# pyani-plus/pyani-plus

Measured on AMD Instinct MI355X. Metric: pairwise genome comparisons/sec (N x N ANI matrix), higher is better.
Workload: dtype u64

## Files before the change

### include/pyani_hip.h

```cpp
#ifndef PYANI_HIP_H
#define PYANI_HIP_H

#include <stddef.h>
#include <stdint.h>

#ifdef __cplusplus
extern "C" {
#endif

#define PA_ABI_VERSION 5

#define PA_API __attribute__((visibility("default")))

typedef enum pa_status {
  PA_OK = 0,
  PA_E_INVALID = -1,
  PA_E_HIP = -2,
  PA_E_NOMEM = -3,
  PA_E_CAPACITY = -4,
  PA_E_NODEVICE = -5,
  PA_E_IO = -6,
  PA_E_NOCONVERGE = -7
} pa_status;

// ... 31 lines not shown
PA_API int pa_fasta_batch_load(const char *const *paths, uint32_t n, int threads, pa_fasta_batch **out);
PA_API int pa_fasta_batch_info(const pa_fasta_batch *batch, uint32_t i, char md5hex33[33], uint64_t *n_residues,
                        uint64_t *n_records, uint64_t *n_invalid, uint64_t *n_bases, uint64_t *n_text,
                        const char **description, const char **message, int *was_gzip);
PA_API int pa_fasta_batch_records(const pa_fasta_batch *batch, uint32_t i, const uint64_t **rec_start,
                           const uint64_t **rec_len, uint64_t *n_records);
PA_API uint64_t pa_fasta_batch_arena_bases(const pa_fasta_batch *batch);
PA_API int pa_fasta_batch_copy_arena(const pa_fasta_batch *batch, uint32_t *h_packed, uint32_t *h_mask,
                              uint64_t *h_genome_start);
PA_API void pa_fasta_batch_free(pa_fasta_batch *batch);

PA_API uint64_t pa_max_hash(uint64_t scaled);

PA_API int pa_arena_dirty(pa_ctx *ctx, const uint32_t *d_mask, uint64_t arena_bases, uint64_t *d_dirty);

PA_API int pa_sketch(pa_ctx *ctx, const uint32_t *d_packed, const uint32_t *d_mask, const uint64_t *d_dirty,
              uint64_t arena_bases, const uint64_t *h_genome_start, uint32_t n_genomes, uint32_t k, uint64_t max_hash,
              uint64_t *d_hashes, uint64_t cap_hashes, uint64_t *d_off, uint64_t *h_total);

PA_API int64_t pa_mask_runs(const uint32_t *h_mask, uint64_t arena_bases, uint64_t *h_run_start, uint64_t *h_run_len,
                            uint64_t cap);
PA_API int pa_mask_from_runs(pa_ctx *ctx, const uint64_t *h_run_start, const uint64_t *h_run_len, uint32_t n_runs,
                             uint32_t *d_mask, uint64_t arena_bases);
PA_API int pa_sketch_streamed(pa_ctx *ctx, const uint32_t *h_packed, const uint64_t *h_run_start,
                              const uint64_t *h_run_len, uint32_t n_runs, uint64_t arena_bases,
                              const uint64_t *h_genome_start, uint32_t n_genomes, uint32_t k, uint64_t max_hash,
                              uint32_t *d_packed, uint32_t *d_mask, uint64_t *d_dirty, uint64_t *d_hashes,
                              uint64_t cap_hashes, uint64_t *d_off, uint64_t *h_total);

#define PA_PAIRS_AUTO 0
#define PA_PAIRS_BITROW 1
#define PA_PAIRS_MERGE 2
#define PA_PAIRS_BITROW_HASH 3
PA_API int pa_pair_counts(pa_ctx *ctx, const uint64_t *d_hashes, const uint64_t *d_off, uint32_t n,
                   uint32_t q0, uint32_t q1, uint32_t s0, uint32_t s1, uint32_t *d_counts, int algo);
PA_API int pa_pair_counts_ex(pa_ctx *ctx, const uint64_t *d_hashes, const uint64_t *d_off, const uint64_t *h_off,
                      uint32_t n, uint32_t q0, uint32_t q1, uint32_t s0, uint32_t s1, uint32_t *d_counts, int algo);
PA_API int pa_pair_dict_prepare(pa_ctx *ctx, const uint64_t *d_subject_hashes, uint64_t n_postings);

PA_API int pa_ani(pa_ctx *ctx, const uint32_t *d_counts, const uint64_t *d_off, uint32_t q0, uint32_t q1,
           uint32_t s0, uint32_t s1, uint32_t k, double *d_identity, double *d_cov_query);
PA_API int pa_ani_host(const uint32_t *h_counts, const uint64_t *h_q_sizes, const uint64_t *h_s_sizes,
                uint32_t nq, uint32_t ns, uint32_t k, double *h_identity, double *h_cov_query,
                uint8_t *h_is_null, int symmetric, uint32_t n_threads);

PA_API int pa_sketch_bottom(pa_ctx *ctx, const uint32_t *d_packed, const uint32_t *d_mask, const uint64_t *d_dirty, uint64_t arena_bases,
                     const uint64_t *h_genome_start, uint32_t n_genomes, uint32_t k, uint32_t m, uint64_t *d_hashes,
                     uint64_t cap_hashes, uint64_t *d_off, uint64_t *h_total);
PA_API int pa_pair_mash(pa_ctx *ctx, const uint64_t *d_hashes, const uint64_t *d_off, uint32_t n, uint32_t q0, uint32_t q1,
                 uint32_t s0, uint32_t s1, uint32_t m, uint32_t *d_common, uint32_t *d_denom);
PA_API int pa_ani_mash(pa_ctx *ctx, const uint32_t *d_common, const uint32_t *d_denom, uint64_t n_pairs, uint32_t k,
                double *d_ani);

PA_API int pa_fragani(pa_ctx *ctx, const uint32_t *d_packed, const uint32_t *d_mask, uint64_t arena_bases,
               const uint64_t *h_contig_start, const uint32_t *h_contig_len, const uint32_t *h_contig_genome,
               uint32_t n_contigs, uint32_t n_genomes, uint32_t k, uint32_t frag_len, uint32_t ref0, uint32_t ref1,
               uint32_t *h_total_frags, uint32_t *h_matched, double *h_ident_sum);
#define PA_FRAGANI_REUSE_INDEX 1u
#define PA_FRAGANI_COLUMNS_ONLY 2u
PA_API int pa_fragani_ex(pa_ctx *ctx, const uint32_t *d_packed, const uint32_t *d_mask, uint64_t arena_bases,
                  const uint64_t *h_contig_start, const uint32_t *h_contig_len, const uint32_t *h_contig_genome,
                  uint32_t n_contigs, uint32_t n_genomes, uint32_t k, uint32_t frag_len, uint32_t qry0, uint32_t qry1,
                  uint32_t ref0, uint32_t ref1, uint32_t flags, uint32_t *h_total_frags, uint32_t *h_matched,
                  double *h_ident_sum);
PA_API int pa_fragani_workspace(pa_ctx *ctx, uint64_t *held_bytes, uint64_t *peak_bytes, uint64_t *cap_bytes);
PA_API int pa_fragani_set_workspace_cap(pa_ctx *ctx, uint64_t cap_bytes);
// ... 231 lines not shown
```

### pyani_plus_amd/_capi.py

```python

from __future__ import annotations

import ctypes as C
import os
import subprocess
from pathlib import Path

_PKG = Path(__file__).resolve().parent
LIB_PATH = _PKG / "_lib" / "libpyani_hip.so"
TOOLS_LIB_PATH = _PKG / "_lib" / "libpyani_hip_tools.so"

ABI_VERSION = 5
PA_OK = 0
PA_E_INVALID = -1
PA_E_NOMEM = -3
PA_E_CAPACITY = -4
PA_E_IO = -6
PA_E_NOCONVERGE = -7
PA_MUL_TALL_MAX_P = 32
PA_EIGS_MAX_K = 24
PA_MANTEL_MAX_N = 16384
PA_MANTEL_LANES = 64
PA_MANTEL_BATCH = 256
PA_MSA_BOOT_BATCH = 32
PA_DEREP_GREEDY, PA_DEREP_COVER = 0, 1
PA_DEREP_MODE = {"greedy": PA_DEREP_GREEDY, "cover": PA_DEREP_COVER}
PA_DEREP_BATCH = 64
PA_DEREP_NONE = 0xFFFFFFFF
PA_SIG_UNHANDLED = 1
PA_FRAGANI_REUSE_INDEX = 1
PA_FRAGANI_COLUMNS_ONLY = 2
PA_PAIRS_AUTO, PA_PAIRS_BITROW, PA_PAIRS_MERGE, PA_PAIRS_BITROW_HASH = 0, 1, 2, 3
PA_ALIGN_BASES = 64
PA_SELECT_MAX_RANKS = 8
PA_KDE_CHAIN = 2048
PA_HIST_WIDE_LDS_BINS = 8192
PA_BIN2D_MAX_BINS = 1024
PA_BIN2D_LDS_CELLS = 4096
PA_BIN2D_SLOTS = 2048
PA_BIN2D_NONE = 0xFFFFFFFFFFFFFFFF
PA_TETRA_BINS = 336
PA_TETRA_WORDS = 256
PROF_PHASES = {"kmer_hash": 0, "sketch_sort": 1, "pair_dict": 2, "pair_count": 3, "ani": 4, "frag_index": 5, "frag_seed": 6, "frag_map": 7,
               "msa_pack": 8, "msa_pairs": 9, "cls_edges": 10, "cls_sort": 11, "rowdist": 12, "nj_scan": 13, "nj_join": 14, "nj_update": 15,
               "msa_boot": 16, "msa_boot_dist": 17}
PA_AGG = {"min": 0, "max": 1, "mean": 2}

_u8p = C.POINTER(C.c_uint8)
_u32p = C.POINTER(C.c_uint32)
_u64p = C.POINTER(C.c_uint64)
_f64p = C.POINTER(C.c_double)
_vp = C.c_void_p

SIGNATURES: dict[str, tuple] = {
    "pa_abi_version": (C.c_int, []),
    "pa_last_error": (C.c_char_p, []),
    "pa_device_count": (C.c_int, []),
    "pa_ctx_create": (C.c_int, [C.c_int, C.POINTER(_vp)]),
    "pa_ctx_destroy": (None, [_vp]),
    "pa_ctx_set_stream": (C.c_int, [_vp, _vp]),
    "pa_ctx_own_stream": (C.c_int, [_vp]),
    "pa_ctx_sync": (C.c_int, [_vp]),
    "pa_ctx_device_info": (C.c_int, [_vp, C.c_char_p, C.POINTER(C.c_int), _u64p]),
    "pa_dev_alloc": (C.c_int, [_vp, C.c_uint64, C.POINTER(_vp)]),
    "pa_dev_free": (C.c_int, [_vp, _vp]),
# ... 233 lines not shown
```

### pyani_plus_amd/csrc/capi.hip

```cpp
#include <algorithm>
#include <cstdarg>
#include <cstring>

#include "pa_internal.h"

static thread_local char g_err[1024] = "";

void pa_set_error(const char *fmt, ...) {
  va_list ap;
  va_start(ap, fmt);
  vsnprintf(g_err, sizeof(g_err), fmt, ap);
  va_end(ap);
}

static hipEvent_t take_event(pa_ctx *c) {
  if (!c->event_pool.empty()) {
    hipEvent_t e = c->event_pool.back();
    c->event_pool.pop_back();
    return e;
  }
  hipEvent_t e = nullptr;
  if (hipEventCreate(&e) != hipSuccess) return nullptr;
  return e;
}
// ... 232 lines not shown
    uint64_t *keys[2] = {c->cand_keys[0].as<uint64_t>(), c->cand_keys[1].as<uint64_t>()};
    uint32_t *vals[2] = {c->cand_vals[0].as<uint32_t>(), c->cand_vals[1].as<uint32_t>()};
    int which = 0;
    int hash_bits = max_hash ? 64 - __builtin_clzll(max_hash) : 0;
    hash_bits = (hash_bits + 7) & ~7;
    int genome_bits = n_genomes > 1 ? 32 - __builtin_clz(n_genomes - 1) : 0;
    genome_bits = (genome_bits + 7) & ~7;
    PA_TRY(pa_radix_sort_pairs(c, keys, vals, n_cand, 0, hash_bits, false, &which));
    PA_TRY(pa_radix_sort_pairs(c, keys, vals, n_cand, 0, genome_bits, true, &which));
    int st = pa_build_sketch_csr(c, keys[which], vals[which], n_cand, n_genomes, d_hashes, cap_hashes, d_off, h_total);
    if (st != PA_OK) return st;
  }
  return PA_OK;
}

extern "C" {

int pa_sketch(pa_ctx *c, const uint32_t *d_packed, const uint32_t *d_mask, const uint64_t *d_dirty_in, uint64_t arena_bases,
              const uint64_t *h_genome_start, uint32_t n_genomes, uint32_t k, uint64_t max_hash, uint64_t *d_hashes,
              uint64_t cap_hashes, uint64_t *d_off, uint64_t *h_total) {
  PA_REQUIRE(c && d_off && h_total && h_genome_start, "pa_sketch: null argument");
  PA_REQUIRE(arena_bases == 0 || (d_packed && d_mask), "pa_sketch: null arena");
  SketchPlan plan;
  PA_TRY(pa_sketch_plan(h_genome_start, n_genomes, arena_bases, k, max_hash, "pa_sketch", &plan));
  PA_HIP(hipSetDevice(c->device));
  return pa_sketch_resident(c, d_packed, d_mask, d_dirty_in, plan, k, max_hash, d_hashes, cap_hashes, d_off, h_total);
}

int pa_pair_counts_ex(pa_ctx *c, const uint64_t *d_hashes, const uint64_t *d_off, const uint64_t *h_off, uint32_t n,
                      uint32_t q0, uint32_t q1, uint32_t s0, uint32_t s1, uint32_t *d_counts, int algo) {
  PA_REQUIRE(c && d_off, "pa_pair_counts: null argument");
  PA_REQUIRE(q0 <= q1 && q1 <= n && s0 <= s1 && s1 <= n, "pa_pair_counts: ranges [%u,%u) x [%u,%u) outside [0,%u)", q0,
             q1, s0, s1, n);
  PA_REQUIRE(algo == PA_PAIRS_AUTO || algo == PA_PAIRS_BITROW || algo == PA_PAIRS_MERGE || algo == PA_PAIRS_BITROW_HASH,
             "pa_pair_counts: unknown algo %d", algo);
  PA_HIP(hipSetDevice(c->device));
  if (q0 == q1 || s0 == s1) { c->dict_prepared = false; return PA_OK; }
  PA_REQUIRE(d_counts != nullptr, "pa_pair_counts: null counts buffer");
  uint64_t total = 0;
  if (h_off) {
    total = h_off[n];
  } else {
    PA_TRY(pa_read_back(c, d_off + n, &total));
  }
  PA_REQUIRE(total == 0 || d_hashes, "pa_pair_counts: null hashes");
  if (algo != PA_PAIRS_AUTO && algo != PA_PAIRS_BITROW_HASH) c->dict_prepared = false;
  switch (algo) {
    case PA_PAIRS_AUTO:
    case PA_PAIRS_BITROW_HASH:
      return pa_pairs_bitrow_hash(c, d_hashes, d_off, h_off, n, total, q0, q1, s0, s1, d_counts);
    case PA_PAIRS_BITROW:
      return pa_pairs_bitrow(c, d_hashes, d_off, n, total, q0, q1, s0, s1, d_counts);
    case PA_PAIRS_MERGE:
      return pa_pairs_merge(c, d_hashes, d_off, n, q0, q1, s0, s1, d_counts);
    default:
      pa_set_error("pa_pair_counts: unknown algo %d", algo);
      return PA_E_INVALID;
  }
}

int pa_pair_counts(pa_ctx *c, const uint64_t *d_hashes, const uint64_t *d_off, uint32_t n, uint32_t q0, uint32_t q1,
                   uint32_t s0, uint32_t s1, uint32_t *d_counts, int algo) {
  return pa_pair_counts_ex(c, d_hashes, d_off, nullptr, n, q0, q1, s0, s1, d_counts, algo);
}

int pa_pair_dict_prepare(pa_ctx *c, const uint64_t *d_subject_hashes, uint64_t n_postings) {
  PA_REQUIRE(c && (n_postings == 0 || d_subject_hashes), "pa_pair_dict_prepare: null argument");
  PA_HIP(hipSetDevice(c->device));
  return pa_pair_dict_prepare_impl(c, d_subject_hashes, n_postings);
}

int pa_ani(pa_ctx *c, const uint32_t *d_counts, const uint64_t *d_off, uint32_t q0, uint32_t q1, uint32_t s0,
           uint32_t s1, uint32_t k, double *d_identity, double *d_cov_query) {
  PA_REQUIRE(c && d_counts && d_off && d_identity && d_cov_query, "pa_ani: null argument");
  PA_REQUIRE(k >= 1 && q0 <= q1 && s0 <= s1, "pa_ani: bad k or ranges");
  PA_HIP(hipSetDevice(c->device));
  return pa_launch_ani(c, d_counts, d_off, q0, q1, s0, s1, k, d_identity, d_cov_query);
}

int pa_prof_enable(pa_ctx *c, int on) {
  PA_REQUIRE(c != nullptr, "null context");
  c->prof_on = on != 0;
  return PA_OK;
// ... 57 lines not shown
```

### pyani_plus_amd/csrc/pa_internal.h

```cpp
#pragma once

#include <hip/hip_runtime.h>

#include <algorithm>
#include <cstdarg>
#include <cstdint>
#include <cstdio>
#include <cstring>
#include <initializer_list>
#include <string>
#include <type_traits>
#include <vector>

#include "../../include/pyani_hip.h"
#include "pa_launch_geom.h"

void pa_set_error(const char *fmt, ...);

#define PA_HIP(call)                                                                          \
  do {                                                                                        \
    hipError_t _e = (call);                                                                   \
    if (_e != hipSuccess) {                                                                   \
      pa_set_error("%s failed: %s (%s:%d)", #call, hipGetErrorString(_e), __FILE__, __LINE__); \
      return PA_E_HIP;                                                                        \
// ... 78 lines not shown

struct ScalarSlot {
  uint32_t word, words;
  constexpr uint32_t bytes() const { return words * 4u; }
  constexpr bool apart_from(ScalarSlot o) const { return word + words <= o.word || o.word + o.words <= word; }
};
constexpr bool slots_apart(uint32_t region_bytes, std::initializer_list<ScalarSlot> slots) {
  for (const ScalarSlot *a = slots.begin(); a != slots.end(); ++a) {
    if ((a->word + a->words) * 4u > region_bytes || (a->words % 2 == 0 && a->word % 2)) return false;
    for (const ScalarSlot *b = a + 1; b != slots.end(); ++b)
      if (!a->apart_from(*b)) return false;
  }
  return true;
}

constexpr uint32_t kCtxScalarBytes = 128;
constexpr ScalarSlot kCandCount{0, 2};
constexpr ScalarSlot kSketchTotal{2, 2};
constexpr ScalarSlot kDenseIds{4, 4};
constexpr uint32_t kDenseOr = 0, kDenseDistinct = 1;
constexpr ScalarSlot kCompactTotal{8, 2};
constexpr ScalarSlot kRegionOverflow{12, 1};
constexpr ScalarSlot kNjPick{16, 8};
constexpr ScalarSlot kDistBad{24, 8};
constexpr ScalarSlot kDerepProgress{14, 2};
static_assert(slots_apart(kCtxScalarBytes, {kCandCount, kSketchTotal, kDenseIds, kCompactTotal, kRegionOverflow, kNjPick, kDistBad, kDerepProgress}),
              "two slots of pa_ctx::counters overlap or leave the block");

constexpr uint32_t kDictScalarBytes = 64;
constexpr ScalarSlot kDictCounters{0, 2};
constexpr uint32_t kDictIdCounter = 0, kDictSpecialId = 1;
constexpr ScalarSlot kDictPreparedFp{2, 4};
constexpr ScalarSlot kDictTileFp{6, 4};
static_assert(slots_apart(kDictScalarBytes, {kDictCounters, kDictPreparedFp, kDictTileFp}),
              "two slots of pa_ctx::dict_scalars overlap or leave the block");

constexpr uint32_t kPinnedBytes = 64;

#define PA_CTX_BUFFERS(ONE, PAIR)                                                                                   \
  PAIR(cand_keys) PAIR(cand_vals) ONE(genome_blk) ONE(counters) ONE(hist) ONE(flags) ONE(scan_tmp) ONE(region_off) \
  ONE(region_cursor) ONE(dirty) PAIR(dict_keys) PAIR(dict_vals) ONE(ids) ONE(post_genome) ONE(bitrows)             \
  ONE(dict_scalars) ONE(cls_i) ONE(cls_j) ONE(cls_score) ONE(cls_cov) ONE(bin2d) ONE(tetra_tab) ONE(nj_work) ONE(pcoa_work) \
  ONE(mantel_work) ONE(derep_work) ONE(boot_work)

struct pa_ctx {
  int device = 0;
  hipStream_t stream = nullptr;
  bool own_stream = false;
  hipDeviceProp_t prop;
#define PA_ONE(name) DevBuf name;
#define PA_PAIR(name) DevBuf name[2];
  PA_CTX_BUFFERS(PA_ONE, PA_PAIR)
#undef PA_ONE
#undef PA_PAIR
  template <class Fn>
  void each_buffer(Fn &&fn) {
#define PA_ONE(name) fn(name);
#define PA_PAIR(name) fn(name[0]); fn(name[1]);
    PA_CTX_BUFFERS(PA_ONE, PA_PAIR)
#undef PA_ONE
#undef PA_PAIR
  }
  template <typename T = uint32_t>
  T *slot(ScalarSlot s) const { return reinterpret_cast<T *>(counters.as<uint32_t>() + s.word); }
  template <typename T = uint32_t>
  T *dict_slot(ScalarSlot s) const { return reinterpret_cast<T *>(dict_scalars.as<uint32_t>() + s.word); }
  bool dict_prepared = false;
  uint64_t dict_prepared_postings = 0;
  uint32_t dict_prepared_cap = 0;
  hipStream_t copy_stream = nullptr;
  void *frag_work = nullptr;
  uint64_t *h_pinned = nullptr;
  bool prof_on = false;
  ProfPhase prof[PA_PROF_NPHASES];
  std::vector<hipEvent_t> event_pool;
// ... 152 lines not shown
      const uint64_t room = (uint64_t)((double)(h_genome_start[g + 1] - s) * plan->frac * 1.25) + 128;
      plan->longest_region = std::max(plan->longest_region, room);
      plan->region_off[g + 1] = plan->region_off[g] + room;
    }
  }
  PA_REQUIRE(plan->n_blocks < (1ULL << 32), "%s: arena too large", who);
  return PA_OK;
}
int pa_regions_begin(pa_ctx *c, const SketchPlan &plan);
CandSink pa_region_sink(pa_ctx *c, uint32_t n_genomes);
int pa_sketch_resident(pa_ctx *c, const uint32_t *d_packed, const uint32_t *d_mask, const uint64_t *d_dirty_in,
                       const SketchPlan &plan, uint32_t k, uint64_t max_hash, uint64_t *d_hashes, uint64_t cap_hashes,
                       uint64_t *d_off, uint64_t *h_total);

int pa_build_dirty(pa_ctx *c, const uint32_t *d_mask, uint64_t n_blocks64, uint64_t *d_dirty, hipStream_t stream = nullptr);
int pa_dirty_or_build(pa_ctx *c, const uint32_t *d_mask, uint64_t n_blocks64, const uint64_t *d_dirty, const uint64_t **out);

constexpr uint32_t kLdsSortMax = 16384;
int pa_sketch_from_regions(pa_ctx *c, uint64_t *d_regions, const uint64_t *d_region_off, const uint32_t *d_cursor,
                           const uint32_t *d_overflow, uint32_t n_genomes, uint32_t longest_region, uint64_t max_hash,
                           uint64_t *d_hashes, uint64_t cap_hashes, uint64_t *d_off, uint64_t *h_total, bool *h_overflow);

int pa_build_sketch_csr(pa_ctx *c, const uint64_t *d_sorted_hash, const uint32_t *d_sorted_genome,
                        uint64_t n_cand, uint32_t n_genomes, uint64_t *d_hashes, uint64_t cap_hashes,
                        uint64_t *d_off, uint64_t *h_total);

int pa_pairs_bitrow(pa_ctx *c, const uint64_t *d_hashes, const uint64_t *d_off, uint32_t n, uint64_t total,
                    uint32_t q0, uint32_t q1, uint32_t s0, uint32_t s1, uint32_t *d_counts);
int pa_dense_ids_sorted(pa_ctx *c, const uint64_t *d_hashes, const uint64_t *d_off, uint32_t n, uint64_t P,
                        uint64_t *n_distinct);
int pa_pairs_bitrow_hash(pa_ctx *c, const uint64_t *d_hashes, const uint64_t *d_off, const uint64_t *h_off ,
                         uint32_t n, uint64_t total, uint32_t q0, uint32_t q1, uint32_t s0, uint32_t s1,
                         uint32_t *d_counts);
int pa_pair_dict_prepare_impl(pa_ctx *c, const uint64_t *d_subject_hashes, uint64_t n_postings);
int pa_pairs_merge(pa_ctx *c, const uint64_t *d_hashes, const uint64_t *d_off, uint32_t n, uint32_t q0,
                   uint32_t q1, uint32_t s0, uint32_t s1, uint32_t *d_counts);

int pa_launch_ani(pa_ctx *c, const uint32_t *d_counts, const uint64_t *d_off, uint32_t q0, uint32_t q1,
                  uint32_t s0, uint32_t s1, uint32_t k, double *d_identity, double *d_cov_query);
```

### pyani_plus_amd/csrc/pairs_bitrow.hip

```cpp
#include <algorithm>
#include <cstdlib>
#include <vector>

#include "pa_internal.h"

namespace {

constexpr int kThreads = 256;
constexpr int kPlanes = 10;
constexpr uint32_t kMaxTileSubjects = 2048;
constexpr uint32_t kNone = 0xffffffffu;
constexpr uint64_t kEmptyKey = ~0ULL;

__global__ __launch_bounds__(kThreads) void iota_kernel(uint32_t *__restrict__ vals, uint64_t n) {
  const uint64_t i = (uint64_t)blockIdx.x * kThreads + threadIdx.x;
  if (i < n) vals[i] = (uint32_t)i;
}

__global__ __launch_bounds__(kThreads) void last_or_kernel(const uint64_t *__restrict__ hashes,
                                                           const uint64_t *__restrict__ off, uint32_t n,
                                                           unsigned long long *__restrict__ or_out) {
  const uint32_t g = blockIdx.x * kThreads + threadIdx.x;
  uint64_t k = 0;
  if (g < n && off[g + 1] > off[g]) k = hashes[off[g + 1] - 1];
// ... 204 lines not shown

template <bool SET_BITS>
__global__ __launch_bounds__(kThreads) void table_lookup_kernel(
    const uint64_t *__restrict__ hashes, uint64_t p0, uint64_t p1, const DictEntry *__restrict__ table, uint32_t cap,
    const uint32_t *__restrict__ special, uint32_t *__restrict__ ids_csr, const uint64_t *__restrict__ off, uint32_t n,
    uint32_t t0, uint32_t w32, uint32_t *__restrict__ rows) {
  uint64_t p;
  if constexpr (SET_BITS) {
    const uint64_t beg = off[t0 + blockIdx.y];
    p = beg + (uint64_t)blockIdx.x * kThreads + threadIdx.x;
    if (p >= off[t0 + blockIdx.y + 1]) return;
  } else {
    p = p0 + (uint64_t)blockIdx.x * kThreads + threadIdx.x;
    if (p >= p1) return;
  }
  const uint64_t h = hashes[p];
  uint32_t id = kNone;
  if (h == kEmptyKey) {
    id = special[0];
  } else {
    uint32_t slot = slot_of(h, cap);
    for (;;) {
      const uint4 e = *reinterpret_cast<const uint4 *>(&table[slot]);
      const uint64_t k = ((uint64_t)e.y << 32) | e.x;
      if (k == h) { id = e.z; break; }
      if (k == kEmptyKey) break;
      if (++slot == cap) slot = 0;
    }
  }
  ids_csr[p] = id;
  if constexpr (SET_BITS) {
    const uint32_t col = blockIdx.y;
    atomicOr(&rows[(uint64_t)id * w32 + (col >> 5)], 1u << (col & 31u));
  }
}

__global__ __launch_bounds__(kThreads) void postings_fingerprint_kernel(const uint64_t *__restrict__ hashes, uint64_t n,
                                                                        unsigned long long *__restrict__ out) {
  uint64_t a = 0, b = 0;
  for (uint64_t i = (uint64_t)blockIdx.x * kThreads + threadIdx.x; i < n; i += (uint64_t)gridDim.x * kThreads) {
    const uint64_t h = hashes[i];
    a += h;
    b += (h ^ (h >> 29)) * 0x9E3779B97F4A7C15ULL;
  }
#pragma unroll
  for (int o = 32; o > 0; o >>= 1) { a += __shfl_xor(a, o, 64); b += __shfl_xor(b, o, 64); }
  if ((threadIdx.x & 63u) == 0) {
    atomicAdd(&out[0], (unsigned long long)a);
    atomicAdd(&out[1], (unsigned long long)b);
  }
}

__global__ __launch_bounds__(256) void mirror_lower_kernel(uint32_t *__restrict__ counts, uint32_t n, uint32_t tile) {
  __shared__ uint32_t s_t[32][33];
  const uint32_t r0 = blockIdx.y * 32u, c0 = blockIdx.x * 32u;
  if (r0 / tile <= c0 / tile) return;
  const uint32_t tx = threadIdx.x & 31u, ty = threadIdx.x >> 5;
  for (uint32_t y = ty; y < 32u; y += 8u) {
    const uint32_t sr = c0 + y, sc = r0 + tx;
    s_t[y][tx] = (sr < n && sc < n) ? counts[(uint64_t)sr * n + sc] : 0u;
  }
  __syncthreads();
  for (uint32_t y = ty; y < 32u; y += 8u) {
    const uint32_t dr = r0 + y, dc = c0 + tx;
    if (dr < n && dc < n) counts[(uint64_t)dr * n + dc] = s_t[tx][y];
  }
// ... 87 lines not shown


static int dict_insert(pa_ctx *c, const uint64_t *d_postings, uint64_t n_post, uint32_t *cap_out) {
  const uint64_t cap64 = n_post + n_post / 2 + 1024;
  PA_REQUIRE(cap64 < (1ULL << 32), "pair phase: tile with %llu subject postings is too large for the hash dictionary",
             (unsigned long long)n_post);
  PA_TRY(c->dict_scalars.reserve(kDictScalarBytes));
  uint32_t *d_counter = c->dict_slot(kDictCounters) + kDictIdCounter, *d_special = c->dict_slot(kDictCounters) + kDictSpecialId;
  PA_TRY(c->dict_keys[0].reserve(cap64 * sizeof(DictEntry)));
  PA_HIP(hipMemsetAsync(c->dict_keys[0].p, 0xff, cap64 * sizeof(DictEntry), c->stream));
  PA_HIP(hipMemsetAsync(d_counter, 0, 4, c->stream));
  PA_HIP(hipMemsetAsync(d_special, 0xff, 4, c->stream));
  PA_TRY(PA_LAUNCH(c, table_insert_kernel, ceil_div(n_post, kThreads * kInsertPerThread), kThreads, 0, d_postings, (uint64_t)0, n_post,
                   c->dict_keys[0].as<DictEntry>(), (uint32_t)cap64, d_counter, d_special));
  *cap_out = (uint32_t)cap64;
  return PA_OK;
}

int pa_pair_dict_prepare_impl(pa_ctx *c, const uint64_t *d_subject_hashes, uint64_t n_postings) {
  ProfScope prof(c, PA_PROF_PAIR_DICT);
  c->dict_prepared = false;
  uint32_t cap = 0;
  PA_TRY(dict_insert(c, d_subject_hashes, n_postings, &cap));
  unsigned long long *d_fp = c->dict_slot<unsigned long long>(kDictPreparedFp);
  PA_HIP(hipMemsetAsync(d_fp, 0, kDictPreparedFp.bytes(), c->stream));
  PA_TRY(PA_LAUNCH(c, postings_fingerprint_kernel, std::min<uint64_t>(1024u, ceil_div(n_postings, kThreads)), kThreads, 0, d_subject_hashes,
                   n_postings, d_fp));
  c->dict_prepared = true;
  c->dict_prepared_postings = n_postings;
  c->dict_prepared_cap = cap;
  return PA_OK;
}

int pa_pairs_bitrow_hash(pa_ctx *c, const uint64_t *d_hashes, const uint64_t *d_off, const uint64_t *h_off_in,
                         uint32_t n, uint64_t total, uint32_t q0, uint32_t q1, uint32_t s0, uint32_t s1,
                         uint32_t *d_counts) {
  const uint32_t nq = q1 - q0, ns = s1 - s0;
  const bool prepared = c->dict_prepared;
  c->dict_prepared = false;
  if (nq == 0 || ns == 0) return PA_OK;
  if (total == 0) {
    PA_HIP(hipMemsetAsync(d_counts, 0, (uint64_t)nq * ns * sizeof(uint32_t), c->stream));
    return PA_OK;
  }
  PA_REQUIRE(total < (1ULL << 32), "pair phase: %llu postings exceed the 32-bit index space", (unsigned long long)total);
  std::vector<uint64_t> h_off_own;
  const uint64_t *h_off = h_off_in;
  if (!h_off) {
    h_off_own.resize(n + 1);
    PA_TRY(pa_copy_to_host(c, h_off_own.data(), d_off, (uint64_t)(n + 1) * 8));
    h_off = h_off_own.data();
  }
  PA_TRY(c->ids.reserve(total * sizeof(uint32_t)));
  PA_TRY(c->dict_scalars.reserve(kDictScalarBytes));
  uint32_t *d_ids = c->ids.as<uint32_t>();
  uint32_t *d_counter = c->dict_slot(kDictCounters) + kDictIdCounter, *d_special = c->dict_slot(kDictCounters) + kDictSpecialId;
  PA_REQUIRE(!prepared || ns <= kMaxTileSubjects, "pair phase: a prepared dictionary serves one tile of at most %u subjects",
             kMaxTileSubjects);
  static const bool symmetry_off = [] { const char *v = PA_TOOL_ENV("PA_PAIRS_SYMMETRIC"); return v && v[0] == '0'; }();
  const bool symmetric = !symmetry_off && q0 == s0 && q1 == s1 && ns > kMaxTileSubjects;
  for (uint32_t t0 = s0; t0 < s1; t0 += kMaxTileSubjects) {
    const uint32_t t1 = (s1 - t0 > kMaxTileSubjects) ? t0 + kMaxTileSubjects : s1;
    const uint32_t cols = t1 - t0;
    const int tpr = (int)((cols + 127u) / 128u);
    const uint32_t w32 = (uint32_t)tpr * 4u;
    const uint32_t tq1 = symmetric ? t1 : q1;
    const uint64_t pt0 = h_off[t0], pt1 = h_off[t1], pq0 = h_off[q0], pq1 = h_off[tq1];
    uint32_t cap = 0;
    {
      ProfScope prof(c, PA_PROF_PAIR_DICT);
      if (prepared) {
        PA_REQUIRE(c->dict_prepared_postings == pt1 - pt0,
                   "pair phase: the prepared dictionary holds %llu postings, the subject tile has %llu",
                   (unsigned long long)c->dict_prepared_postings, (unsigned long long)(pt1 - pt0));
        unsigned long long *d_tile_fp = c->dict_slot<unsigned long long>(kDictTileFp);
        PA_HIP(hipMemsetAsync(d_tile_fp, 0, kDictTileFp.bytes(), c->stream));
        PA_TRY(PA_LAUNCH(c, postings_fingerprint_kernel, std::min<uint64_t>(1024u, ceil_div(pt1 - pt0, kThreads)), kThreads, 0, d_hashes + pt0,
                         pt1 - pt0, d_tile_fp));
        unsigned long long fp_prepared[2], fp_tile[2];
        ReadBack rb(c);
        PA_TRY(rb.queue(c->dict_slot<unsigned long long>(kDictPreparedFp), fp_prepared, 2));
        PA_TRY(rb.queue(d_tile_fp, fp_tile, 2));
        PA_TRY(rb.wait());
        PA_REQUIRE(fp_prepared[0] == fp_tile[0] && fp_prepared[1] == fp_tile[1],
                   "pair phase: the prepared dictionary was built from other postings than the subject tile's "
                   "(same count, %llu, different content)", (unsigned long long)(pt1 - pt0));
        cap = c->dict_prepared_cap;
      } else {
        PA_TRY(dict_insert(c, d_hashes + pt0, pt1 - pt0, &cap));
      }
      constexpr uint64_t kRowBoundBytes = 4ULL << 30;
      uint64_t row_bound = (pt1 - pt0) ? (pt1 - pt0) : 1;
      if (row_bound * w32 * sizeof(uint32_t) > kRowBoundBytes && row_bound * w32 * sizeof(uint32_t) > c->bitrows.bytes) {
        uint32_t distinct = 0;
        PA_TRY(pa_read_back(c, d_counter, &distinct));
        row_bound = std::max<uint64_t>(1, std::min<uint64_t>(row_bound, distinct));
      }
      PA_TRY(c->bitrows.reserve(row_bound * w32 * sizeof(uint32_t)));
      PA_TRY(PA_LAUNCH(c, zero_rows_kernel, ceil_div(row_bound * w32 / 4u, kThreads), kThreads, 0, c->bitrows.as<uint4>(), d_counter, w32));
      const DictEntry *table = c->dict_keys[0].as<DictEntry>();
      if (pt1 > pt0) {
        uint64_t longest = 0;
        for (uint32_t g = t0; g < t1; ++g) longest = std::max(longest, h_off[g + 1] - h_off[g]);
        PA_TRY(PA_LAUNCH(c, table_lookup_kernel<true>, LaunchDim(ceil_div(longest, kThreads), cols), kThreads, 0, d_hashes, pt0, pt1, table, cap,
                         d_special, d_ids, d_off, n, t0, w32, c->bitrows.as<uint32_t>()));
      }
      const uint64_t a0 = pq0, a1 = pq1 < pt0 ? pq1 : pt0;
      const uint64_t b0 = pq0 > pt1 ? pq0 : pt1, b1 = pq1;
      if (a1 > a0)
        PA_TRY(PA_LAUNCH(c, table_lookup_kernel<false>, ceil_div(a1 - a0, kThreads), kThreads, 0, d_hashes, a0, a1, table, cap, d_special, d_ids,
                         d_off, n, t0, w32, nullptr));
      if (b1 > b0)
        PA_TRY(PA_LAUNCH(c, table_lookup_kernel<false>, ceil_div(b1 - b0, kThreads), kThreads, 0, d_hashes, b0, b1, table, cap, d_special, d_ids,
                         d_off, n, t0, w32, nullptr));
    }
    {
      ProfScope prof(c, PA_PROF_PAIR_COUNT);
      const uint32_t *rows = c->bitrows.as<uint32_t>();
      PA_TRY(dispatch_row_sum(c, tpr, tq1 - q0, d_ids, d_off, q0, rows, cols, d_counts, ns, t0 - s0));
    }
  }
  if (symmetric) {
    ProfScope prof(c, PA_PROF_PAIR_COUNT);
    static_assert(kMaxTileSubjects % 32u == 0, "mirror pieces must not straddle a tile edge");
    const uint32_t g = (ns + 31u) / 32u;
    PA_TRY(PA_LAUNCH(c, mirror_lower_kernel, LaunchDim(g, g), 256, 0, d_counts, ns, kMaxTileSubjects));
  }
  return PA_OK;
}
```

Baseline: 87.11 million.

## Build pair dictionary per hash-range bucket in LDS instead of global hash table

```diff
diff --git a/include/pyani_hip.h b/include/pyani_hip.h
--- a/include/pyani_hip.h
+++ b/include/pyani_hip.h
@@ -87,6 +87,7 @@
 #define PA_PAIRS_BITROW 1
 #define PA_PAIRS_MERGE 2
 #define PA_PAIRS_BITROW_HASH 3
+#define PA_PAIRS_BITROW_BUCKET 4
 PA_API int pa_pair_counts(pa_ctx *ctx, const uint64_t *d_hashes, const uint64_t *d_off, uint32_t n,
                    uint32_t q0, uint32_t q1, uint32_t s0, uint32_t s1, uint32_t *d_counts, int algo);
 PA_API int pa_pair_counts_ex(pa_ctx *ctx, const uint64_t *d_hashes, const uint64_t *d_off, const uint64_t *h_off,
diff --git a/pyani_plus_amd/_capi.py b/pyani_plus_amd/_capi.py
--- a/pyani_plus_amd/_capi.py
+++ b/pyani_plus_amd/_capi.py
@@ -30,7 +30,7 @@
 PA_SIG_UNHANDLED = 1
 PA_FRAGANI_REUSE_INDEX = 1
 PA_FRAGANI_COLUMNS_ONLY = 2
-PA_PAIRS_AUTO, PA_PAIRS_BITROW, PA_PAIRS_MERGE, PA_PAIRS_BITROW_HASH = 0, 1, 2, 3
+PA_PAIRS_AUTO, PA_PAIRS_BITROW, PA_PAIRS_MERGE, PA_PAIRS_BITROW_HASH, PA_PAIRS_BITROW_BUCKET = 0, 1, 2, 3, 4
 PA_ALIGN_BASES = 64
 PA_SELECT_MAX_RANKS = 8
 PA_KDE_CHAIN = 2048
diff --git a/pyani_plus_amd/csrc/capi.hip b/pyani_plus_amd/csrc/capi.hip
--- a/pyani_plus_amd/csrc/capi.hip
+++ b/pyani_plus_amd/csrc/capi.hip
@@ -288,7 +288,8 @@
   PA_REQUIRE(c && d_off, "pa_pair_counts: null argument");
   PA_REQUIRE(q0 <= q1 && q1 <= n && s0 <= s1 && s1 <= n, "pa_pair_counts: ranges [%u,%u) x [%u,%u) outside [0,%u)", q0,
              q1, s0, s1, n);
-  PA_REQUIRE(algo == PA_PAIRS_AUTO || algo == PA_PAIRS_BITROW || algo == PA_PAIRS_MERGE || algo == PA_PAIRS_BITROW_HASH,
+  PA_REQUIRE(algo == PA_PAIRS_AUTO || algo == PA_PAIRS_BITROW || algo == PA_PAIRS_MERGE || algo == PA_PAIRS_BITROW_HASH ||
+                 algo == PA_PAIRS_BITROW_BUCKET,
              "pa_pair_counts: unknown algo %d", algo);
   PA_HIP(hipSetDevice(c->device));
   if (q0 == q1 || s0 == s1) { c->dict_prepared = false; return PA_OK; }
@@ -303,8 +304,12 @@
   if (algo != PA_PAIRS_AUTO && algo != PA_PAIRS_BITROW_HASH) c->dict_prepared = false;
   switch (algo) {
     case PA_PAIRS_AUTO:
+      if (!c->dict_prepared) return pa_pairs_bitrow_bucket(c, d_hashes, d_off, h_off, n, total, q0, q1, s0, s1, d_counts);
+      [[fallthrough]];
     case PA_PAIRS_BITROW_HASH:
       return pa_pairs_bitrow_hash(c, d_hashes, d_off, h_off, n, total, q0, q1, s0, s1, d_counts);
+    case PA_PAIRS_BITROW_BUCKET:
+      return pa_pairs_bitrow_bucket(c, d_hashes, d_off, h_off, n, total, q0, q1, s0, s1, d_counts);
     case PA_PAIRS_BITROW:
       return pa_pairs_bitrow(c, d_hashes, d_off, n, total, q0, q1, s0, s1, d_counts);
     case PA_PAIRS_MERGE:
diff --git a/pyani_plus_amd/csrc/pa_internal.h b/pyani_plus_amd/csrc/pa_internal.h
--- a/pyani_plus_amd/csrc/pa_internal.h
+++ b/pyani_plus_amd/csrc/pa_internal.h
@@ -134,7 +134,9 @@
 constexpr uint32_t kDictIdCounter = 0, kDictSpecialId = 1;
 constexpr ScalarSlot kDictPreparedFp{2, 4};
 constexpr ScalarSlot kDictTileFp{6, 4};
-static_assert(slots_apart(kDictScalarBytes, {kDictCounters, kDictPreparedFp, kDictTileFp}),
+constexpr ScalarSlot kDictBucketRule{10, 4};
+constexpr ScalarSlot kDictBucketOverflow{14, 1};
+static_assert(slots_apart(kDictScalarBytes, {kDictCounters, kDictPreparedFp, kDictTileFp, kDictBucketRule, kDictBucketOverflow}),
               "two slots of pa_ctx::dict_scalars overlap or leave the block");
 
 constexpr uint32_t kPinnedBytes = 64;
@@ -142,7 +144,7 @@
 #define PA_CTX_BUFFERS(ONE, PAIR)                                                                                   \
   PAIR(cand_keys) PAIR(cand_vals) ONE(genome_blk) ONE(counters) ONE(hist) ONE(flags) ONE(scan_tmp) ONE(region_off) \
   ONE(region_cursor) ONE(dirty) PAIR(dict_keys) PAIR(dict_vals) ONE(ids) ONE(post_genome) ONE(bitrows)             \
-  ONE(dict_scalars) ONE(cls_i) ONE(cls_j) ONE(cls_score) ONE(cls_cov) ONE(bin2d) ONE(tetra_tab) ONE(nj_work) ONE(pcoa_work) \
+  ONE(dict_scalars) ONE(run_bounds) ONE(cls_i) ONE(cls_j) ONE(cls_score) ONE(cls_cov) ONE(bin2d) ONE(tetra_tab) ONE(nj_work) ONE(pcoa_work) \
   ONE(mantel_work) ONE(derep_work) ONE(boot_work)
 
 struct pa_ctx {
@@ -361,6 +363,9 @@
 int pa_pairs_bitrow_hash(pa_ctx *c, const uint64_t *d_hashes, const uint64_t *d_off, const uint64_t *h_off ,
                          uint32_t n, uint64_t total, uint32_t q0, uint32_t q1, uint32_t s0, uint32_t s1,
                          uint32_t *d_counts);
+int pa_pairs_bitrow_bucket(pa_ctx *c, const uint64_t *d_hashes, const uint64_t *d_off, const uint64_t *h_off ,
+                           uint32_t n, uint64_t total, uint32_t q0, uint32_t q1, uint32_t s0, uint32_t s1,
+                           uint32_t *d_counts);
 int pa_pair_dict_prepare_impl(pa_ctx *c, const uint64_t *d_subject_hashes, uint64_t n_postings);
 int pa_pairs_merge(pa_ctx *c, const uint64_t *d_hashes, const uint64_t *d_off, uint32_t n, uint32_t q0,
                    uint32_t q1, uint32_t s0, uint32_t s1, uint32_t *d_counts);
diff --git a/pyani_plus_amd/csrc/pairs_bitrow.hip b/pyani_plus_amd/csrc/pairs_bitrow.hip
--- a/pyani_plus_amd/csrc/pairs_bitrow.hip
+++ b/pyani_plus_amd/csrc/pairs_bitrow.hip
@@ -260,6 +260,182 @@
   if constexpr (SET_BITS) {
     const uint32_t col = blockIdx.y;
     atomicOr(&rows[(uint64_t)id * w32 + (col >> 5)], 1u << (col & 31u));
+  }
+}
+
+constexpr uint32_t kBucketThreads = 1024;
+constexpr uint32_t kBucketSlots = 8192;
+constexpr uint32_t kBucketMaxDistinct = kBucketSlots / 3 * 2;
+constexpr uint32_t kBucketMeanPostings = kBucketSlots / 4;
+constexpr uint64_t kRunBoundsMaxBytes = 1ULL << 30;
+static_assert(kBucketMaxDistinct + kBucketThreads < kBucketSlots, "the probe of a bucket's LDS table must always find an empty slot");
+static_assert((kBucketSlots & (kBucketSlots - 1)) == 0, "the LDS probe wraps with a mask");
+static_assert(kBucketSlots * 12u + 64u <= 160u * 1024u, "the table of a bucket fits the 160 KB of a CU's LDS");
+
+struct BucketRule {
+  unsigned long long key_max;
+  uint32_t shift, mult;
+};
+static_assert(sizeof(BucketRule) == kDictBucketRule.bytes(), "the rule fills its slot");
+
+__device__ __forceinline__ uint32_t bucket_of(uint64_t h, uint32_t shift, uint32_t mult, uint32_t n_buckets) {
+  const uint32_t b = (uint32_t)(((h >> shift) * (uint64_t)mult) >> 32);
+  return b < n_buckets ? b : n_buckets - 1u;
+}
+
+__global__ __launch_bounds__(kBucketThreads) void bucket_rule_kernel(const uint64_t *__restrict__ hashes,
+                                                                     const uint64_t *__restrict__ off, uint32_t g_lo,
+                                                                     uint32_t n_g, uint32_t n_buckets,
+                                                                     BucketRule *__restrict__ rule,
+                                                                     uint32_t *__restrict__ overflow) {
+  __shared__ unsigned long long s_max[kBucketThreads / 64];
+  uint64_t k = 0;
+  for (uint32_t g = threadIdx.x; g < n_g; g += kBucketThreads) {
+    const uint64_t beg = off[g_lo + g], end = off[g_lo + g + 1];
+    const uint64_t last = end > beg ? hashes[end - 1] : 0;
+    k = last > k ? last : k;
+  }
+#pragma unroll
+  for (int o = 32; o > 0; o >>= 1) {
+    const uint64_t other = __shfl_xor(k, o, 64);
+    k = other > k ? other : k;
+  }
+  if ((threadIdx.x & 63u) == 0) s_max[threadIdx.x >> 6] = k;
+  __syncthreads();
+  if (threadIdx.x != 0) return;
+  for (uint32_t w = 1; w < kBucketThreads / 64; ++w) k = s_max[w] > k ? (uint64_t)s_max[w] : k;
+  const int key_bits = k ? 64 - __builtin_clzll(k) : 1;
+  const uint32_t shift = key_bits > 32 ? (uint32_t)key_bits - 32u : 0u;
+  const uint64_t top = (k >> shift) + 1;
+  const uint64_t mult = ((uint64_t)n_buckets << 32) / top;
+  rule->key_max = k;
+  rule->shift = shift;
+  rule->mult = mult < 0xffffffffull ? (uint32_t)mult : 0xffffffffu;
+  *overflow = 0;
+}
+
+__global__ __launch_bounds__(kThreads) void run_bounds_kernel(const uint64_t *__restrict__ hashes,
+                                                              const uint64_t *__restrict__ off, uint32_t g_lo,
+                                                              uint32_t n_g, uint32_t n_buckets,
+                                                              const BucketRule *__restrict__ rule,
+                                                              uint32_t *__restrict__ bounds) {
+  const uint32_t g = blockIdx.x;
+  const uint64_t beg = off[g_lo + g], end = off[g_lo + g + 1];
+  uint32_t *__restrict__ col = bounds + g;
+  if (beg == end) {
+    if (blockIdx.y == 0)
+      for (uint32_t b = threadIdx.x; b <= n_buckets; b += kThreads) col[(uint64_t)b * n_g] = (uint32_t)beg;
+    return;
+  }
+  const uint64_t p = beg + (uint64_t)blockIdx.y * kThreads + threadIdx.x;
+  if (p >= end) return;
+  const uint32_t shift = rule->shift, mult = rule->mult;
+  const uint32_t mine = bucket_of(hashes[p], shift, mult, n_buckets);
+  const uint32_t first = p == beg ? 0u : bucket_of(hashes[p - 1], shift, mult, n_buckets) + 1u;
+  for (uint32_t b = first; b <= mine; ++b) col[(uint64_t)b * n_g] = (uint32_t)p;
+  if (p + 1 == end)
+    for (uint32_t b = mine + 1u; b <= n_buckets; ++b) col[(uint64_t)b * n_g] = (uint32_t)end;
+}
+
+__device__ __forceinline__ uint32_t lds_slot_of(uint64_t h) {
+  const uint32_t x = ((uint32_t)h * 0x9E3779B1u) ^ (uint32_t)(h >> 32);
+  return (x * 0x85EBCA6Bu) >> (32 - __builtin_ctz(kBucketSlots));
+}
+
+struct BucketTile {
+  const uint64_t *hashes;
+  const uint32_t *bounds;
+  uint32_t n_g;
+  uint32_t s_lo, n_subjects;
+  uint32_t qa_lo, n_qa;
+  uint32_t qb_lo, n_qb;
+  uint32_t w32;
+  uint32_t *rows, *ids_csr;
+  uint32_t *counter, *overflow;
+};
+
+__global__ __launch_bounds__(kBucketThreads) void bucket_dict_kernel(const BucketTile t) {
+  __shared__ unsigned long long s_key[kBucketSlots];
+  __shared__ uint32_t s_id[kBucketSlots];
+  __shared__ uint32_t s_count, s_special, s_over, s_base;
+  const uint32_t tid = threadIdx.x;
+  for (uint32_t x = tid; x < kBucketSlots; x += kBucketThreads) s_key[x] = kEmptyKey;
+  if (tid == 0) { s_count = 0; s_special = kNone; s_over = 0; }
+  __syncthreads();
+  const uint32_t *__restrict__ run_lo = t.bounds + (uint64_t)blockIdx.x * t.n_g;
+  const uint32_t *__restrict__ run_hi = run_lo + t.n_g;
+
+  for (uint32_t g = tid; g < t.n_subjects; g += kBucketThreads) {
+    const uint32_t p1 = run_hi[t.s_lo + g];
+    for (uint32_t p = run_lo[t.s_lo + g]; p < p1; ++p) {
+      if (*(volatile uint32_t *)&s_over) break;
+      const uint64_t h = t.hashes[p];
+      uint32_t won = kNone;
+      if (h == kEmptyKey) {
+        if (atomicCAS(&s_special, kNone, kNone - 1u) == kNone) won = kBucketSlots;
+      } else {
+        uint32_t slot = lds_slot_of(h);
+        for (;;) {
+          unsigned long long k = *(volatile unsigned long long *)&s_key[slot];
+          if (k == kEmptyKey) k = atomicCAS(&s_key[slot], (unsigned long long)kEmptyKey, (unsigned long long)h);
+          if (k == kEmptyKey) { won = slot; break; }
+          if (k == h) break;
+          slot = (slot + 1u) & (kBucketSlots - 1u);
+        }
+      }
+      if (won != kNone) {
+        const uint32_t local = atomicAdd(&s_count, 1u);
+        if (local >= kBucketMaxDistinct) *(volatile uint32_t *)&s_over = 1;
+        if (won == kBucketSlots) s_special = local; else s_id[won] = local;
+      }
+    }
+  }
+  __syncthreads();
+  if (s_over) {
+    if (tid == 0) atomicOr(t.overflow, 1u);
+    return;
+  }
+  const uint32_t distinct = s_count;
+  if (tid == 0) s_base = distinct ? atomicAdd(t.counter, distinct) : 0u;
+  __syncthreads();
+  const uint32_t base = s_base;
+  uint4 *mine = reinterpret_cast<uint4 *>(t.rows + (uint64_t)base * t.w32);
+  for (uint32_t x = tid; x < distinct * (t.w32 / 4u); x += kBucketThreads) mine[x] = make_uint4(0u, 0u, 0u, 0u);
+  __syncthreads();
+
+  auto id_of = [&](uint64_t h) -> uint32_t {
+    if (h == kEmptyKey) return s_special == kNone ? kNone : base + s_special;
+    uint32_t slot = lds_slot_of(h);
+    for (;;) {
+      const unsigned long long k = s_key[slot];
+      if (k == h) return base + s_id[slot];
+      if (k == kEmptyKey) return kNone;
+      slot = (slot + 1u) & (kBucketSlots - 1u);
+    }
+  };
+  for (uint32_t g = tid; g < t.n_subjects; g += kBucketThreads) {
+    const uint32_t p1 = run_hi[t.s_lo + g];
+    for (uint32_t p = run_lo[t.s_lo + g]; p < p1; ++p) {
+      const uint32_t id = id_of(t.hashes[p]);
+      t.ids_csr[p] = id;
+      const uint32_t lane = tid & 63u;
+      const uint64_t active = __ballot(1);
+      const uint32_t before = __shfl_up(id, 1, 64);
+      const bool head = (lane & 31u) == 0 || !((active >> (lane - 1u)) & 1u) || before != id;
+      const uint64_t stops = (__ballot(head) | ~active) & ~((2ULL << lane) - 1ULL);
+      uint32_t end = stops ? (uint32_t)__builtin_ctzll(stops) : 64u;
+      end = end < (lane | 31u) + 1u ? end : (lane | 31u) + 1u;
+      if (head && id != kNone) {
+        const uint32_t n_bits = end - lane;
+        const uint32_t bits = (n_bits == 32u ? ~0u : (1u << n_bits) - 1u) << (lane & 31u);
+        atomicOr(&t.rows[(uint64_t)id * t.w32 + (g >> 5)], bits);
+      }
+    }
+  }
+  for (uint32_t x = tid; x < t.n_qa + t.n_qb; x += kBucketThreads) {
+    const uint32_t g = x < t.n_qa ? t.qa_lo + x : t.qb_lo + (x - t.n_qa);
+    const uint32_t p1 = run_hi[g];
+    for (uint32_t p = run_lo[g]; p < p1; ++p) t.ids_csr[p] = id_of(t.hashes[p]);
   }
 }
 
@@ -413,9 +589,129 @@
   return PA_OK;
 }
 
-int pa_pairs_bitrow_hash(pa_ctx *c, const uint64_t *d_hashes, const uint64_t *d_off, const uint64_t *h_off_in,
-                         uint32_t n, uint64_t total, uint32_t q0, uint32_t q1, uint32_t s0, uint32_t s1,
-                         uint32_t *d_counts) {
+namespace {
+
+struct PairCall {
+  const uint64_t *d_hashes, *d_off, *h_off;
+  uint32_t n, q0;
+};
+struct PairTile {
+  uint32_t t0, t1, cols, w32, tq1;
+  uint64_t pt0, pt1, pq0, pq1;
+  uint64_t row_bound() const { return pt1 > pt0 ? pt1 - pt0 : 1; }
+};
+
+constexpr uint64_t kRowBoundBytes = 4ULL << 30;
+bool rows_need_the_count(const pa_ctx *c, const PairTile &t) {
+  const uint64_t bytes = t.row_bound() * t.w32 * sizeof(uint32_t);
+  return bytes > kRowBoundBytes && bytes > c->bitrows.bytes;
+}
+
+int hash_tile_dict(pa_ctx *c, const PairCall &k, const PairTile &t, bool prepared) {
+  ProfScope prof(c, PA_PROF_PAIR_DICT);
+  const uint64_t *d_hashes = k.d_hashes;
+  uint32_t *d_ids = c->ids.as<uint32_t>();
+  uint32_t *d_counter = c->dict_slot(kDictCounters) + kDictIdCounter, *d_special = c->dict_slot(kDictCounters) + kDictSpecialId;
+  const uint64_t pt0 = t.pt0, pt1 = t.pt1;
+  uint32_t cap = 0;
+  if (prepared) {
+    PA_REQUIRE(c->dict_prepared_postings == pt1 - pt0,
+               "pair phase: the prepared dictionary holds %llu postings, the subject tile has %llu",
+               (unsigned long long)c->dict_prepared_postings, (unsigned long long)(pt1 - pt0));
+    unsigned long long *d_tile_fp = c->dict_slot<unsigned long long>(kDictTileFp);
+    PA_HIP(hipMemsetAsync(d_tile_fp, 0, kDictTileFp.bytes(), c->stream));
+    PA_TRY(PA_LAUNCH(c, postings_fingerprint_kernel, std::min<uint64_t>(1024u, ceil_div(pt1 - pt0, kThreads)), kThreads, 0, d_hashes + pt0,
+                     pt1 - pt0, d_tile_fp));
+    unsigned long long fp_prepared[2], fp_tile[2];
+    ReadBack rb(c);
+    PA_TRY(rb.queue(c->dict_slot<unsigned long long>(kDictPreparedFp), fp_prepared, 2));
+    PA_TRY(rb.queue(d_tile_fp, fp_tile, 2));
+    PA_TRY(rb.wait());
+    PA_REQUIRE(fp_prepared[0] == fp_tile[0] && fp_prepared[1] == fp_tile[1],
+               "pair phase: the prepared dictionary was built from other postings than the subject tile's "
+               "(same count, %llu, different content)", (unsigned long long)(pt1 - pt0));
+    cap = c->dict_prepared_cap;
+  } else {
+    PA_TRY(dict_insert(c, d_hashes + pt0, pt1 - pt0, &cap));
+  }
+  uint64_t row_bound = t.row_bound();
+  if (rows_need_the_count(c, t)) {
+    uint32_t distinct = 0;
+    PA_TRY(pa_read_back(c, d_counter, &distinct));
+    row_bound = std::max<uint64_t>(1, std::min<uint64_t>(row_bound, distinct));
+  }
+  PA_TRY(c->bitrows.reserve(row_bound * t.w32 * sizeof(uint32_t)));
+  PA_TRY(PA_LAUNCH(c, zero_rows_kernel, ceil_div(row_bound * t.w32 / 4u, kThreads), kThreads, 0, c->bitrows.as<uint4>(), d_counter, t.w32));
+  const DictEntry *table = c->dict_keys[0].as<DictEntry>();
+  if (pt1 > pt0) {
+    uint64_t longest = 0;
+    for (uint32_t g = t.t0; g < t.t1; ++g) longest = std::max(longest, k.h_off[g + 1] - k.h_off[g]);
+    PA_TRY(PA_LAUNCH(c, table_lookup_kernel<true>, LaunchDim(ceil_div(longest, kThreads), t.cols), kThreads, 0, d_hashes, pt0, pt1, table, cap,
+                     d_special, d_ids, k.d_off, k.n, t.t0, t.w32, c->bitrows.as<uint32_t>()));
+  }
+  const uint64_t a0 = t.pq0, a1 = t.pq1 < pt0 ? t.pq1 : pt0;
+  const uint64_t b0 = t.pq0 > pt1 ? t.pq0 : pt1, b1 = t.pq1;
+  if (a1 > a0)
+    PA_TRY(PA_LAUNCH(c, table_lookup_kernel<false>, ceil_div(a1 - a0, kThreads), kThreads, 0, d_hashes, a0, a1, table, cap, d_special, d_ids,
+                     k.d_off, k.n, t.t0, t.w32, nullptr));
+  if (b1 > b0)
+    PA_TRY(PA_LAUNCH(c, table_lookup_kernel<false>, ceil_div(b1 - b0, kThreads), kThreads, 0, d_hashes, b0, b1, table, cap, d_special, d_ids,
+                     k.d_off, k.n, t.t0, t.w32, nullptr));
+  return PA_OK;
+}
+
+struct BucketPlan {
+  uint32_t g_lo = 0, n_g = 0;
+  uint32_t n_buckets = 0;
+};
+
+int bucket_plan(pa_ctx *c, const PairCall &k, uint32_t q1, uint32_t s0, uint32_t s1, BucketPlan *plan) {
+  ProfScope prof(c, PA_PROF_PAIR_DICT);
+  plan->g_lo = std::min(k.q0, s0);
+  plan->n_g = std::max(q1, s1) - plan->g_lo;
+  uint64_t most = 0, longest = 1;
+  for (uint32_t t0 = s0; t0 < s1; t0 += kMaxTileSubjects) most = std::max(most, k.h_off[std::min<uint64_t>(s1, (uint64_t)t0 + kMaxTileSubjects)] - k.h_off[t0]);
+  for (uint32_t g = plan->g_lo; g < plan->g_lo + plan->n_g; ++g) longest = std::max(longest, k.h_off[g + 1] - k.h_off[g]);
+  uint32_t n_buckets = 1;
+  while ((uint64_t)n_buckets * kBucketMeanPostings < most) n_buckets <<= 1;
+  const uint64_t bytes = ((uint64_t)n_buckets + 1) * plan->n_g * sizeof(uint32_t);
+  if (bytes > kRunBoundsMaxBytes) return PA_OK;
+  PA_TRY(c->run_bounds.reserve(bytes));
+  BucketRule *d_rule = c->dict_slot<BucketRule>(kDictBucketRule);
+  PA_TRY(PA_LAUNCH(c, bucket_rule_kernel, 1, kBucketThreads, 0, k.d_hashes, k.d_off, plan->g_lo, plan->n_g, n_buckets, d_rule,
+                   c->dict_slot(kDictBucketOverflow)));
+  PA_TRY(PA_LAUNCH(c, run_bounds_kernel, LaunchDim(plan->n_g, ceil_div(longest, kThreads)), kThreads, 0, k.d_hashes, k.d_off, plan->g_lo, plan->n_g,
+                   n_buckets, d_rule, c->run_bounds.as<uint32_t>()));
+  plan->n_buckets = n_buckets;
+  return PA_OK;
+}
+
+int bucket_tile_dict(pa_ctx *c, const PairCall &k, const PairTile &t, const BucketPlan &plan) {
+  ProfScope prof(c, PA_PROF_PAIR_DICT);
+  uint32_t *d_counter = c->dict_slot(kDictCounters) + kDictIdCounter;
+  PA_TRY(c->bitrows.reserve(t.row_bound() * t.w32 * sizeof(uint32_t)));
+  PA_HIP(hipMemsetAsync(d_counter, 0, 4, c->stream));
+  BucketTile b;
+  b.hashes = k.d_hashes;
+  b.bounds = c->run_bounds.as<uint32_t>();
+  b.n_g = plan.n_g;
+  b.s_lo = t.t0 - plan.g_lo;
+  b.n_subjects = t.cols;
+  const uint32_t a1 = std::min(t.tq1, t.t0), b0 = std::max(k.q0, t.t1);
+  b.qa_lo = k.q0 - plan.g_lo;
+  b.n_qa = a1 > k.q0 ? a1 - k.q0 : 0;
+  b.qb_lo = b0 - plan.g_lo;
+  b.n_qb = t.tq1 > b0 ? t.tq1 - b0 : 0;
+  b.w32 = t.w32;
+  b.rows = c->bitrows.as<uint32_t>();
+  b.ids_csr = c->ids.as<uint32_t>();
+  b.counter = d_counter;
+  b.overflow = c->dict_slot(kDictBucketOverflow);
+  return PA_LAUNCH(c, bucket_dict_kernel, plan.n_buckets, kBucketThreads, 0, b);
+}
+
+int pairs_bitrow_tiles(pa_ctx *c, const uint64_t *d_hashes, const uint64_t *d_off, const uint64_t *h_off_in, uint32_t n, uint64_t total,
+                       uint32_t q0, uint32_t q1, uint32_t s0, uint32_t s1, uint32_t *d_counts, bool by_buckets) {
   const uint32_t nq = q1 - q0, ns = s1 - s0;
   const bool prepared = c->dict_prepared;
   c->dict_prepared = false;
@@ -435,71 +731,33 @@
   PA_TRY(c->ids.reserve(total * sizeof(uint32_t)));
   PA_TRY(c->dict_scalars.reserve(kDictScalarBytes));
   uint32_t *d_ids = c->ids.as<uint32_t>();
-  uint32_t *d_counter = c->dict_slot(kDictCounters) + kDictIdCounter, *d_special = c->dict_slot(kDictCounters) + kDictSpecialId;
   PA_REQUIRE(!prepared || ns <= kMaxTileSubjects, "pair phase: a prepared dictionary serves one tile of at most %u subjects",
              kMaxTileSubjects);
+  const PairCall call{d_hashes, d_off, h_off, n, q0};
+  BucketPlan plan;
+  if (by_buckets && !prepared) PA_TRY(bucket_plan(c, call, q1, s0, s1, &plan));
   static const bool symmetry_off = [] { const char *v = PA_TOOL_ENV("PA_PAIRS_SYMMETRIC"); return v && v[0] == '0'; }();
   const bool symmetric = !symmetry_off && q0 == s0 && q1 == s1 && ns > kMaxTileSubjects;
   for (uint32_t t0 = s0; t0 < s1; t0 += kMaxTileSubjects) {
     const uint32_t t1 = (s1 - t0 > kMaxTileSubjects) ? t0 + kMaxTileSubjects : s1;
     const uint32_t cols = t1 - t0;
     const int tpr = (int)((cols + 127u) / 128u);
-    const uint32_t w32 = (uint32_t)tpr * 4u;
     const uint32_t tq1 = symmetric ? t1 : q1;
-    const uint64_t pt0 = h_off[t0], pt1 = h_off[t1], pq0 = h_off[q0], pq1 = h_off[tq1];
-    uint32_t cap = 0;
-    {
-      ProfScope prof(c, PA_PROF_PAIR_DICT);
-      if (prepared) {
-        PA_REQUIRE(c->dict_prepared_postings == pt1 - pt0,
-                   "pair phase: the prepared dictionary holds %llu postings, the subject tile has %llu",
-                   (unsigned long long)c->dict_prepared_postings, (unsigned long long)(pt1 - pt0));
-        unsigned long long *d_tile_fp = c->dict_slot<unsigned long long>(kDictTileFp);
-        PA_HIP(hipMemsetAsync(d_tile_fp, 0, kDictTileFp.bytes(), c->stream));
-        PA_TRY(PA_LAUNCH(c, postings_fingerprint_kernel, std::min<uint64_t>(1024u, ceil_div(pt1 - pt0, kThreads)), kThreads, 0, d_hashes + pt0,
-                         pt1 - pt0, d_tile_fp));
-        unsigned long long fp_prepared[2], fp_tile[2];
-        ReadBack rb(c);
-        PA_TRY(rb.queue(c->dict_slot<unsigned long long>(kDictPreparedFp), fp_prepared, 2));
-        PA_TRY(rb.queue(d_tile_fp, fp_tile, 2));
-        PA_TRY(rb.wait());
-        PA_REQUIRE(fp_prepared[0] == fp_tile[0] && fp_prepared[1] == fp_tile[1],
-                   "pair phase: the prepared dictionary was built from other postings than the subject tile's "
-                   "(same count, %llu, different content)", (unsigned long long)(pt1 - pt0));
-        cap = c->dict_prepared_cap;
-      } else {
-        PA_TRY(dict_insert(c, d_hashes + pt0, pt1 - pt0, &cap));
-      }
-      constexpr uint64_t kRowBoundBytes = 4ULL << 30;
-      uint64_t row_bound = (pt1 - pt0) ? (pt1 - pt0) : 1;
-      if (row_bound * w32 * sizeof(uint32_t) > kRowBoundBytes && row_bound * w32 * sizeof(uint32_t) > c->bitrows.bytes) {
-        uint32_t distinct = 0;
-        PA_TRY(pa_read_back(c, d_counter, &distinct));
-        row_bound = std::max<uint64_t>(1, std::min<uint64_t>(row_bound, distinct));
-      }
-      PA_TRY(c->bitrows.reserve(row_bound * w32 * sizeof(uint32_t)));
-      PA_TRY(PA_LAUNCH(c, zero_rows_kernel, ceil_div(row_bound * w32 / 4u, kThreads), kThreads, 0, c->bitrows.as<uint4>(), d_counter, w32));
-      const DictEntry *table = c->dict_keys[0].as<DictEntry>();
-      if (pt1 > pt0) {
-        uint64_t longest = 0;
-        for (uint32_t g = t0; g < t1; ++g) longest = std::max(longest, h_off[g + 1] - h_off[g]);
-        PA_TRY(PA_LAUNCH(c, table_lookup_kernel<true>, LaunchDim(ceil_div(longest, kThreads), cols), kThreads, 0, d_hashes, pt0, pt1, table, cap,
-                         d_special, d_ids, d_off, n, t0, w32, c->bitrows.as<uint32_t>()));
-      }
-      const uint64_t a0 = pq0, a1 = pq1 < pt0 ? pq1 : pt0;
-      const uint64_t b0 = pq0 > pt1 ? pq0 : pt1, b1 = pq1;
-      if (a1 > a0)
-        PA_TRY(PA_LAUNCH(c, table_lookup_kernel<false>, ceil_div(a1 - a0, kThreads), kThreads, 0, d_hashes, a0, a1, table, cap, d_special, d_ids,
-                         d_off, n, t0, w32, nullptr));
-      if (b1 > b0)
-        PA_TRY(PA_LAUNCH(c, table_lookup_kernel<false>, ceil_div(b1 - b0, kThreads), kThreads, 0, d_hashes, b0, b1, table, cap, d_special, d_ids,
-                         d_off, n, t0, w32, nullptr));
-    }
-    {
+    const PairTile tile{t0, t1, cols, (uint32_t)tpr * 4u, tq1, h_off[t0], h_off[t1], h_off[q0], h_off[tq1]};
+    auto row_sums = [&]() -> int {
       ProfScope prof(c, PA_PROF_PAIR_COUNT);
-      const uint32_t *rows = c->bitrows.as<uint32_t>();
-      PA_TRY(dispatch_row_sum(c, tpr, tq1 - q0, d_ids, d_off, q0, rows, cols, d_counts, ns, t0 - s0));
-    }
+      return dispatch_row_sum(c, tpr, tq1 - q0, d_ids, d_off, q0, c->bitrows.as<uint32_t>(), cols, d_counts, ns, t0 - s0);
+    };
+    const bool buckets = plan.n_buckets != 0 && !rows_need_the_count(c, tile);
+    if (buckets) PA_TRY(bucket_tile_dict(c, call, tile, plan)); else PA_TRY(hash_tile_dict(c, call, tile, prepared));
+    PA_TRY(row_sums());
+    if (!buckets) continue;
+    uint32_t *d_overflow = c->dict_slot(kDictBucketOverflow), overflow = 0;
+    PA_TRY(pa_read_back(c, d_overflow, &overflow));
+    if (!overflow) continue;
+    PA_HIP(hipMemsetAsync(d_overflow, 0, kDictBucketOverflow.bytes(), c->stream));
+    PA_TRY(hash_tile_dict(c, call, tile, false));
+    PA_TRY(row_sums());
   }
   if (symmetric) {
     ProfScope prof(c, PA_PROF_PAIR_COUNT);
@@ -509,3 +767,15 @@
   }
   return PA_OK;
 }
+
+}
+
+int pa_pairs_bitrow_hash(pa_ctx *c, const uint64_t *d_hashes, const uint64_t *d_off, const uint64_t *h_off, uint32_t n,
+                         uint64_t total, uint32_t q0, uint32_t q1, uint32_t s0, uint32_t s1, uint32_t *d_counts) {
+  return pairs_bitrow_tiles(c, d_hashes, d_off, h_off, n, total, q0, q1, s0, s1, d_counts, false);
+}
+
+int pa_pairs_bitrow_bucket(pa_ctx *c, const uint64_t *d_hashes, const uint64_t *d_off, const uint64_t *h_off, uint32_t n,
+                           uint64_t total, uint32_t q0, uint32_t q1, uint32_t s0, uint32_t s1, uint32_t *d_counts) {
+  return pairs_bitrow_tiles(c, d_hashes, d_off, h_off, n, total, q0, q1, s0, s1, d_counts, true);
+}
```

New measurement: 88.63 million (median of 6 runs). +1.7%, better.
